# Fan-Luo/Legal-RAG

Measured on AMD Instinct MI355X. Metric: queries/sec + Recall@10 (hybrid top-10) on UCC-en, higher is better.
Workload: dtype f32 dense (long batches: fp16 first pass, candidates re-scored in f32) / f64 bm25+fusion; 1 GPU; UCC-en 591 chunks, dense(768-d FlatIP)+BM25 hybrid fusion top-10 (BASELINE configs[1]); unique_queries=1168, top_k=10, fusion=rrf_norm_blend w=0.6/0.4 alpha=0.5 rrf_k=60 min_final=0.2

## Files before the change

### legal-rag_amd/csrc/fuse.hip

```cpp
#include "fuse_core.hpp"

#include <cfloat>
#include <cmath>
#include <cstdlib>
#include <cstring>
#include <vector>

namespace amdr {

constexpr int kFuseMax = 3 * AMDR_MAX_K;

__global__ __launch_bounds__(64) void fuse_kernel(amdr_fuse_params_t P, ChanIn c0, ChanIn c1, ChanIn c2, int max_out,
                                                  long long* __restrict__ out_ids, double* __restrict__ out_vals,
                                                  int* __restrict__ out_mask, int* __restrict__ out_count) {
  extern __shared__ __attribute__((aligned(16))) unsigned char fsm[];
  long long* uid = reinterpret_cast<long long*>(fsm);
  double* sc = reinterpret_cast<double*>(uid + max_out);
  double* tot = sc + max_out;
  int* pos0 = reinterpret_cast<int*>(tot + max_out);
  int* pos[3] = {pos0, pos0 + max_out, pos0 + 2 * max_out};
  const int lane = threadIdx.x;
  const int qi = blockIdx.x;
  const ChanIn ch[3] = {c0, c1, c2};
  const double w[3] = {P.w_dense, P.w_bm25, P.w_colbert};

  int n[3];
  double lo[3], hi[3];
#pragma unroll
  for (int c = 0; c < 3; ++c) {
    int cnt = 0;
    double mn = INFINITY, mx = -INFINITY;
    for (int j = lane; j < ch[c].k; j += 64) {
      if (ch[c].ids[(size_t)qi * ch[c].k + j] >= 0) {
        cnt++;
        double s = chan_score(ch[c], qi, j);
        mn = fmin(mn, s);
        mx = fmax(mx, s);
      }
    }
    n[c] = wave_allsum_i32(cnt);
    lo[c] = wave_min(mn);
    hi[c] = wave_max(mx);
  }

  int U = 0;
#pragma unroll
  for (int c = 0; c < 3; ++c) {
    const int U0 = U;
    for (int base = 0; base < n[c]; base += 64) {
      const int j = base + lane;
      const bool v = j < n[c];
      long long my = v ? chan_uid(ch[c], qi, j) : -1;
      int f = -1;
      if (v)
        for (int u = 0; u < U0; ++u)
          if (uid[u] == my) {
            f = u;
            break;
          }
      const bool isnew = v && f < 0;
      const unsigned long long m = __ballot(isnew);
      const unsigned long long lt = (lane == 0) ? 0ull : (m & (~0ull >> (64 - lane)));
      const int idx = isnew ? U + __popcll(lt) : f;
      if (isnew) {
        uid[idx] = my;
        pos[0][idx] = -1;
        pos[1][idx] = -1;
        pos[2][idx] = -1;
      }
      lds_sync();
      if (v) pos[c][idx] = j;
      U += __popcll(m);
      lds_sync();
    }
  }

  const bool wrrf = (P.method == AMDR_FUSE_WRRF);
  double rmn = INFINITY, rmx = -INFINITY;
  for (int u = lane; u < U; u += 64) {
    double t = 0.0;
#pragma unroll
    for (int c = 0; c < 3; ++c) {
      int p = pos[c][u];
      if (p >= 0) {
        double wc = wrrf ? w[c] : 1.0;
        double v = wc * (1.0 / (double)(P.rrf_k + p + 1));
        t = t + v;
      }
    }
    tot[u] = t;
    rmn = fmin(rmn, t);
    rmx = fmax(rmx, t);
  }
  rmn = wave_min(rmn);
  rmx = wave_max(rmx);
  const bool rdeg = (rmx - rmn < 1e-12);

  FuseCtx X;
  X.rmn = rmn;
  X.rmx = rmx;
  X.rdeg = rdeg;
  X.wrrf = wrrf;
#pragma unroll
  for (int c = 0; c < 3; ++c) {
    X.w[c] = w[c];
    X.lo[c] = lo[c];
    X.hi[c] = hi[c];
  }
  auto eval = [&](int u, double (&val)[AMDR_FUSE_NVALS], int& mk) {
    const int pp[3] = {pos[0][u], pos[1][u], pos[2][u]};
    fuse_eval(P, X, tot[u], pp, [&](int c, int p) { return chan_score(ch[c], qi, p); }, val, mk);
  };

  int kept = 0;
  const size_t obase = (size_t)qi * max_out;
  if (U <= 64) {
    double val[AMDR_FUSE_NVALS];
    int mk = 0;
    const int u = lane;
    if (u < U) {
      eval(u, val, mk);
      sc[u] = val[AMDR_FV_SCORE];
    }
    lds_sync();
    if (u < U) {
      const double s = val[AMDR_FV_SCORE];
      int r = 0;
      for (int v2 = 0; v2 < U; ++v2) {
        const double o = sc[v2];
        r += (o > s) || (o == s && v2 < u);
      }
      if (s >= P.min_final_score) kept++;
      out_ids[obase + r] = uid[u];
      out_mask[obase + r] = mk;
#pragma unroll
      for (int x = 0; x < AMDR_FUSE_NVALS; ++x) out_vals[(obase + r) * AMDR_FUSE_NVALS + x] = val[x];
    }
  } else {
    for (int u = lane; u < U; u += 64) {
      double val[AMDR_FUSE_NVALS];
      int mk;
      eval(u, val, mk);
      sc[u] = val[AMDR_FV_SCORE];
    }
    lds_sync();
    for (int u = lane; u < U; u += 64) {
      double val[AMDR_FUSE_NVALS];
      int mk;
      eval(u, val, mk);
      const double s = val[AMDR_FV_SCORE];
      int r = 0;
      for (int v2 = 0; v2 < U; ++v2) {
        const double o = sc[v2];
        r += (o > s) || (o == s && v2 < u);
      }
      if (s >= P.min_final_score) kept++;
      out_ids[obase + r] = uid[u];
      out_mask[obase + r] = mk;
#pragma unroll
      for (int x = 0; x < AMDR_FUSE_NVALS; ++x) out_vals[(obase + r) * AMDR_FUSE_NVALS + x] = val[x];
    }
  }
  kept = wave_allsum_i32(kept);
  for (int r = U + lane; r < max_out; r += 64) {
    out_ids[obase + r] = -1;
    out_mask[obase + r] = 0;
    for (int x = 0; x < AMDR_FUSE_NVALS; ++x) out_vals[(obase + r) * AMDR_FUSE_NVALS + x] = 0.0;
  }
  if (lane == 0) out_count[qi] = kept;
}

template <int W>
__global__ __launch_bounds__(64) void fuse_packed_kernel(amdr_fuse_params_t P, ChanIn c0, ChanIn c1, ChanIn c2, int nq,
                                                         int max_out, long long* __restrict__ out_ids,
                                                         double* __restrict__ out_vals, int* __restrict__ out_mask,
                                                         int* __restrict__ out_count) {
  FusePre none;
  none.have[0] = none.have[1] = none.have[2] = false;
  fuse_packed_body<W, false>(P, c0, c1, c2, nq, max_out, out_ids, out_vals, out_mask, out_count, none, blockIdx.x * (64 / W));
}

static void launch_fuse(const amdr_fuse_params_t& P, const ChanIn& c0, const ChanIn& c1, const ChanIn& c2, int nq,
                        int max_out, long long* ids, double* vals, int* mask, int* count, hipStream_t st) {
  if (max_out <= 16)
    hipLaunchKernelGGL(fuse_packed_kernel<16>, dim3((nq + 3) / 4), dim3(64), 0, st, P, c0, c1, c2, nq, max_out, ids, vals,
                       mask, count);
  else if (max_out <= 32)
    hipLaunchKernelGGL(fuse_packed_kernel<32>, dim3((nq + 1) / 2), dim3(64), 0, st, P, c0, c1, c2, nq, max_out, ids, vals,
                       mask, count);
  else
    hipLaunchKernelGGL(fuse_kernel, dim3(nq), dim3(64), (size_t)max_out * 36, st, P, c0, c1, c2, max_out, ids, vals, mask,
                       count);
}

__global__ __launch_bounds__(64) void rerank_blend_kernel(int max_out, const int* __restrict__ count,
                                                          long long* __restrict__ ids, double* __restrict__ vals,
                                                          int* __restrict__ mask, const double* __restrict__ ce_raw,
                                                          int top_n, double beta, double* __restrict__ out_rerank) {
  extern __shared__ __attribute__((aligned(16))) unsigned char smem[];
  double* svals = reinterpret_cast<double*>(smem);
  double* snew = svals + (size_t)max_out * AMDR_FUSE_NVALS;
  double* snorm = snew + max_out;
  long long* sids = reinterpret_cast<long long*>(snorm + max_out);
  int* smask = reinterpret_cast<int*>(sids + max_out);
  int* spre = smask + max_out;
  const int lane = threadIdx.x, qi = blockIdx.x;
  const size_t base = (size_t)qi * max_out;
  const int cnt = count[qi];
  const int n = cnt < top_n ? cnt : top_n;
  const double nan = __longlong_as_double(0x7ff8000000000000ll);

  for (int r = lane; r < max_out; r += 64) {
    out_rerank[(base + r) * 2 + 0] = nan;
    out_rerank[(base + r) * 2 + 1] = nan;
  }
  if (n <= 0) return;

  double mn = INFINITY, mx = -INFINITY;
  for (int j = lane; j < n; j += 64) {
    double r = ce_raw[(size_t)qi * top_n + j];
    mn = fmin(mn, r);
    mx = fmax(mx, r);
  }
  mn = wave_min(mn);
  mx = wave_max(mx);
  const bool deg = (mx - mn < 1e-12);

  for (int j = lane; j < cnt; j += 64) {
    for (int x = 0; x < AMDR_FUSE_NVALS; ++x) svals[(size_t)j * AMDR_FUSE_NVALS + x] = vals[(base + j) * AMDR_FUSE_NVALS + x];
    sids[j] = ids[base + j];
    smask[j] = mask[base + j];
    double s = svals[(size_t)j * AMDR_FUSE_NVALS + AMDR_FV_SCORE];
    if (j < n) {
      double raw = ce_raw[(size_t)qi * top_n + j];
      double nm = deg ? 0.0 : (raw - mn) / (mx - mn);
      snorm[j] = nm;
      s = (1 - beta) * s + beta * nm;
    }
    snew[j] = s;
  }
  lds_sync();
  for (int j = lane; j < cnt; j += 64) {
    int p = j;
    if (j < n) {
      const double nm = snorm[j];
      p = 0;
      for (int i = 0; i < n; ++i) {
        const double o = snorm[i];
        p += (o > nm) || (o == nm && i < j);
      }
    }
    spre[j] = p;
  }
  lds_sync();
  for (int j = lane; j < cnt; j += 64) {
    const double s = snew[j];
    const int pj = spre[j];
    int r = 0;
    for (int i = 0; i < cnt; ++i) {
      const double o = snew[i];
      r += (o > s) || (o == s && spre[i] < pj);
    }
    ids[base + r] = sids[j];
    mask[base + r] = smask[j];
    for (int x = 0; x < AMDR_FUSE_NVALS; ++x) vals[(base + r) * AMDR_FUSE_NVALS + x] = svals[(size_t)j * AMDR_FUSE_NVALS + x];
    vals[(base + r) * AMDR_FUSE_NVALS + AMDR_FV_SCORE] = s;
    if (j < n) {
      out_rerank[(base + r) * 2 + 0] = ce_raw[(size_t)qi * top_n + j];
      out_rerank[(base + r) * 2 + 1] = snorm[j];
    }
  }
}

static size_t rerank_lds(int max_out) {
  return (size_t)max_out * (AMDR_FUSE_NVALS + 2) * sizeof(double) + (size_t)max_out * sizeof(long long) +
         (size_t)max_out * 2 * sizeof(int);
}

int dense_fuse_plain_launch(const FuseTail& t, int q0, int m, int kd, const float* dense_scores, const int64_t* dense_ids,
                            hipStream_t st) {
  const FuseTailArgs a = fuse_tail_args(t, q0, kd, dense_scores, dense_ids);
  launch_fuse(*t.p, a.c0, a.c1, ChanIn::none(), m, a.mo, a.ids, a.vals, a.mask, a.count, st);
  AMDR_HIP(hipGetLastError());
  return AMDR_OK;
}

}

using namespace amdr;

namespace {

int fuse_check(const amdr_fuse_params_t* p, int nq, int kd, int kb, int kc) {
  AMDR_REQUIRE(p != nullptr, "fuse: null params");
  AMDR_REQUIRE(p->method >= 0 && p->method <= 3, "fuse: unknown method %d", p->method);
  AMDR_REQUIRE(nq >= 0, "fuse: nq=%d", nq);
  AMDR_REQUIRE(kd >= 0 && kd <= AMDR_MAX_K && kb >= 0 && kb <= AMDR_MAX_K && kc >= 0 && kc <= AMDR_MAX_K,
               "fuse: channel depth outside [0,%d]", AMDR_MAX_K);
  AMDR_REQUIRE(kd + kb + kc >= 1, "fuse: all channels empty (max_out would be 0)");
  return AMDR_OK;
}

}

namespace {
struct Arena {
  char* base = nullptr;
  size_t cap = 0, used = 0;
  int device = -1;
  ~Arena() {
    if (base) (void)hipFree(base);
  }
  int begin(int dev, size_t total) {
    if (dev != device || total > cap) {
      if (base) (void)hipFree(base);
      base = nullptr;
      cap = 0;
      size_t want = total < (1u << 20) ? (1u << 20) : total;
      AMDR_HIP(hipMalloc((void**)&base, want));
      cap = want;
      device = dev;
    }
    used = 0;
    return AMDR_OK;
  }
  void* take(size_t bytes) {
    void* p = base + used;
    used += (bytes + 255) & ~(size_t)255;
    return p;
  }
};
inline size_t pad256(size_t b) { return (b + 255) & ~(size_t)255; }
Arena& arena() {
  static thread_local Arena a;
  return a;
}
}

namespace {
struct Pack {
  std::vector<char>& buf;
  size_t used = 0;
  explicit Pack(std::vector<char>& b) : buf(b) {}
  size_t add(const void* src, size_t bytes) {
    size_t off = used;
    used += pad256(bytes);
    if (buf.size() < used) buf.resize(used);
    if (src && bytes) memcpy(buf.data() + off, src, bytes);
    return off;
  }
};
std::vector<char>& host_block() {
  static thread_local std::vector<char> b;
  return b;
}
}

namespace amdr {
__global__ __launch_bounds__(256) void fuse_compact_kernel(const long long* __restrict__ ids, const double* __restrict__ vals,
                                                           const int* __restrict__ mask, const int* __restrict__ count,
                                                           int nq, int max_out, int w, long long* __restrict__ out_rows,
                                                           double* __restrict__ out_scores, int* __restrict__ out_mask,
                                                           int* __restrict__ out_count) {
  const long i = (long)blockIdx.x * 256 + threadIdx.x;
  if (i >= (long)nq * w) return;
  const int q = (int)(i / w), j = (int)(i - (long)q * w);
  const int c = count[q] < w ? count[q] : w;
  const bool keep = j < c;
  const size_t src = (size_t)q * max_out + j;
  out_rows[i] = keep ? ids[src] : -1ll;
  out_scores[i] = keep ? vals[src * AMDR_FUSE_NVALS + AMDR_FV_SCORE] : 0.0;
  out_mask[i] = keep ? mask[src] : 0;
  if (j == 0) out_count[q] = c;
}
}

extern "C" {

int amdr_fuse_device(const amdr_fuse_params_t* p, int32_t nq, const int64_t* dense_ids, const float* dense_scores,
                     int32_t kd, const int64_t* dense_row2uid, const int64_t* bm25_ids, const double* bm25_scores,
                     int32_t kb, const int64_t* bm25_row2uid, const int64_t* colbert_ids, const float* colbert_scores,
                     int32_t kc, const int64_t* colbert_row2uid, int64_t* out_ids, double* out_vals,
                     int32_t* out_mask, int32_t* out_count, int32_t device, void* stream) {
  int rc = fuse_check(p, nq, kd, kb, kc);
  if (rc) return rc;
  AMDR_REQUIRE((kd == 0 || (dense_ids && dense_scores)) && (kb == 0 || (bm25_ids && bm25_scores)) &&
                   (kc == 0 || (colbert_ids && colbert_scores)),
               "fuse: null channel buffer");
  AMDR_REQUIRE(nq == 0 || (out_ids && out_vals && out_mask && out_count), "fuse: null output");
  if (nq == 0) return AMDR_OK;
  AMDR_HIP(hipSetDevice(device));
  ChanIn c0{(const long long*)dense_ids, dense_scores, (const long long*)dense_row2uid, kd, 0};
  ChanIn c1{(const long long*)bm25_ids, bm25_scores, (const long long*)bm25_row2uid, kb, 1};
  ChanIn c2{(const long long*)colbert_ids, colbert_scores, (const long long*)colbert_row2uid, kc, 0};
  launch_fuse(*p, c0, c1, c2, nq, kd + kb + kc, (long long*)out_ids, out_vals, out_mask, out_count, (hipStream_t)stream);
  AMDR_HIP(hipGetLastError());
  return AMDR_OK;
}

int amdr_rerank_blend_device(int32_t nq, int32_t max_out, const int32_t* count, int64_t* ids, double* vals,
                             int32_t* mask, const double* ce_raw, int32_t top_n, double beta, double* out_rerank,
                             int32_t device, void* stream) {
  AMDR_REQUIRE(nq >= 0 && max_out >= 1 && max_out <= kFuseMax, "rerank_blend: bad sizes");
  AMDR_REQUIRE(top_n >= 1, "rerank_blend: top_n=%d", top_n);
  AMDR_REQUIRE(nq == 0 || (count && ids && vals && mask && ce_raw && out_rerank), "rerank_blend: null buffer");
  if (nq == 0) return AMDR_OK;
  AMDR_HIP(hipSetDevice(device));
  size_t lds = rerank_lds(max_out);
  if (lds > 48 * 1024)
    AMDR_HIP(hipFuncSetAttribute((const void*)rerank_blend_kernel, hipFuncAttributeMaxDynamicSharedMemorySize, (int)lds));
  hipLaunchKernelGGL(rerank_blend_kernel, dim3(nq), dim3(64), lds, (hipStream_t)stream, max_out, count,
                     (long long*)ids, vals, mask, ce_raw, top_n, beta, out_rerank);
  AMDR_HIP(hipGetLastError());
  return AMDR_OK;
}

int amdr_fuse_compact_device(int32_t nq, int32_t max_out, int32_t w, const int64_t* ids, const double* vals,
                             const int32_t* mask, const int32_t* count, int64_t* out_rows, double* out_scores,
                             int32_t* out_mask, int32_t* out_count, int32_t device, void* stream) {
  AMDR_REQUIRE(nq >= 0 && max_out >= 1 && w >= 1 && w <= max_out, "fuse_compact: bad sizes (max_out=%d w=%d)", max_out, w);
  if (nq == 0) return AMDR_OK;
  AMDR_REQUIRE(ids && vals && mask && count && out_rows && out_scores && out_mask && out_count, "fuse_compact: null buffer");
  AMDR_HIP(hipSetDevice(device));
  const long total = (long)nq * w;
  hipLaunchKernelGGL(amdr::fuse_compact_kernel, dim3((unsigned)((total + 255) / 256)), dim3(256), 0, (hipStream_t)stream,
                     (const long long*)ids, vals, mask, count, nq, max_out, w, (long long*)out_rows, out_scores, out_mask,
                     out_count);
  AMDR_HIP(hipGetLastError());
  return AMDR_OK;
}

int amdr_fuse(const amdr_fuse_params_t* p, int32_t nq, const int64_t* dense_ids, const double* dense_scores, int32_t kd,
              const int64_t* bm25_ids, const double* bm25_scores, int32_t kb, const int64_t* colbert_ids,
              const double* colbert_scores, int32_t kc, int64_t* out_ids, double* out_vals, int32_t* out_mask,
              int32_t* out_count) {
  int rc = fuse_check(p, nq, kd, kb, kc);
  if (rc) return rc;
  if (nq == 0) return AMDR_OK;
  AMDR_REQUIRE((kd == 0 || (dense_ids && dense_scores)) && (kb == 0 || (bm25_ids && bm25_scores)) &&
                   (kc == 0 || (colbert_ids && colbert_scores)) && out_ids && out_vals && out_mask && out_count,
               "fuse: null buffer");
  int dev = 0;
  AMDR_HIP(hipGetDevice(&dev));
  const size_t q = (size_t)nq, mo = (size_t)(kd + kb + kc);
  Pack in(host_block());
  const size_t o_di = in.add(dense_ids, q * kd * 8), o_ds = in.add(dense_scores, q * kd * 8);
  const size_t o_bi = in.add(bm25_ids, q * kb * 8), o_bs = in.add(bm25_scores, q * kb * 8);
  const size_t o_ci = in.add(colbert_ids, q * kc * 8), o_cs = in.add(colbert_scores, q * kc * 8);
  const size_t in_bytes = in.used;
  const size_t o_oi = in_bytes, o_ov = o_oi + pad256(q * mo * 8), o_om = o_ov + pad256(q * mo * AMDR_FUSE_NVALS * 8),
               o_oc = o_om + pad256(q * mo * 4), total = o_oc + pad256(q * 4);
  if ((rc = arena().begin(dev, total))) return rc;
  char* d = arena().base;
  hipStream_t st = nullptr;
  std::vector<char>& hb = host_block();
  if (hb.size() < total) hb.resize(total);
  AMDR_HIP(hipMemcpyAsync(d, hb.data(), in_bytes, hipMemcpyHostToDevice, st));
  ChanIn c0{(const long long*)(d + o_di), d + o_ds, nullptr, kd, 1};
  ChanIn c1{(const long long*)(d + o_bi), d + o_bs, nullptr, kb, 1};
  ChanIn c2{(const long long*)(d + o_ci), d + o_cs, nullptr, kc, 1};
  launch_fuse(*p, c0, c1, c2, nq, (int)mo, (long long*)(d + o_oi), (double*)(d + o_ov), (int*)(d + o_om),
              (int*)(d + o_oc), st);
  AMDR_HIP(hipGetLastError());
  AMDR_HIP(hipMemcpyAsync(hb.data() + o_oi, d + o_oi, total - o_oi, hipMemcpyDeviceToHost, st));
  AMDR_HIP(hipStreamSynchronize(st));
  memcpy(out_ids, hb.data() + o_oi, q * mo * 8);
  memcpy(out_vals, hb.data() + o_ov, q * mo * AMDR_FUSE_NVALS * 8);
  memcpy(out_mask, hb.data() + o_om, q * mo * 4);
  memcpy(out_count, hb.data() + o_oc, q * 4);
  return AMDR_OK;
}

int amdr_rerank_blend(int32_t nq, int32_t max_out, const int32_t* count, int64_t* ids, double* vals, int32_t* mask,
                      const double* ce_raw, int32_t top_n, double beta, double* out_rerank) {
  AMDR_REQUIRE(nq >= 0 && max_out >= 1 && max_out <= kFuseMax && top_n >= 1, "rerank_blend: bad sizes");
  if (nq == 0) return AMDR_OK;
  AMDR_REQUIRE(count && ids && vals && mask && ce_raw && out_rerank, "rerank_blend: null buffer");
  int dev = 0, rc;
  AMDR_HIP(hipGetDevice(&dev));
  const size_t q = (size_t)nq, mo = (size_t)max_out;
  Pack in(host_block());
  const size_t o_c = in.add(count, q * 4), o_r = in.add(ce_raw, q * top_n * 8);
  const size_t o_i = in.add(ids, q * mo * 8), o_v = in.add(vals, q * mo * AMDR_FUSE_NVALS * 8),
               o_m = in.add(mask, q * mo * 4);
  const size_t in_bytes = in.used;
  const size_t o_o = in_bytes, total = o_o + pad256(q * mo * 16);
  if ((rc = arena().begin(dev, total))) return rc;
  char* d = arena().base;
  hipStream_t st = nullptr;
  std::vector<char>& hb = host_block();
  if (hb.size() < total) hb.resize(total);
  AMDR_HIP(hipMemcpyAsync(d, hb.data(), in_bytes, hipMemcpyHostToDevice, st));
  rc = amdr_rerank_blend_device(nq, max_out, (const int32_t*)(d + o_c), (int64_t*)(d + o_i), (double*)(d + o_v),
                                (int32_t*)(d + o_m), (const double*)(d + o_r), top_n, beta, (double*)(d + o_o), dev, st);
  if (rc) return rc;
  AMDR_HIP(hipMemcpyAsync(hb.data() + o_i, d + o_i, total - o_i, hipMemcpyDeviceToHost, st));
  AMDR_HIP(hipStreamSynchronize(st));
  memcpy(ids, hb.data() + o_i, q * mo * 8);
  memcpy(vals, hb.data() + o_v, q * mo * AMDR_FUSE_NVALS * 8);
  memcpy(mask, hb.data() + o_m, q * mo * 4);
  memcpy(out_rerank, hb.data() + o_o, q * mo * 16);
  return AMDR_OK;
}


}
```

### legal-rag_amd/csrc/fuse_core.hpp

```cpp
#pragma once
#include "common.hpp"
#include "topk.hpp"

#include <cmath>

namespace amdr {

__device__ __forceinline__ double wave_min(double v) { return wave_allmin_f64(v); }
__device__ __forceinline__ double wave_max(double v) { return wave_allmax_f64(v); }
__device__ __forceinline__ void lds_sync() {
  __builtin_amdgcn_fence(__ATOMIC_ACQ_REL, "wavefront");
  __builtin_amdgcn_wave_barrier();
}

struct ChanIn {
  const long long* ids;
  const void* scores;
  const long long* row2uid;
  int k;
  int is_f64;
  __host__ __device__ static ChanIn none() { return ChanIn{nullptr, nullptr, nullptr, 0, 0}; }
};

__device__ __forceinline__ double chan_score(const ChanIn& c, int qi, int j) {
  size_t off = (size_t)qi * c.k + j;
  return c.is_f64 ? ((const double*)c.scores)[off] : (double)((const float*)c.scores)[off];
}
__device__ __forceinline__ long long chan_uid(const ChanIn& c, int qi, int j) {
  long long id = c.ids[(size_t)qi * c.k + j];
  if (id >= 0 && c.row2uid) id = c.row2uid[id];
  return id;
}

struct FuseCtx {
  double rmn, rmx;
  bool rdeg, wrrf;
  double w[3], lo[3], hi[3];
};
template <class ScoreAt>
__device__ __forceinline__ void fuse_eval(const amdr_fuse_params_t& P, const FuseCtx& X, double t, const int (&pos)[3],
                                          ScoreAt&& score_at, double (&val)[AMDR_FUSE_NVALS], int& mk) {
  const double rrf_norm = X.rdeg ? 0.0 : (t - X.rmn) / (X.rmx - X.rmn);
  double nrm[3], raw[3], wt[3];
  mk = 0;
#pragma unroll
  for (int c = 0; c < 3; ++c) {
    const int p = pos[c];
    nrm[c] = 0.0;
    raw[c] = 0.0;
    if (p >= 0) {
      mk |= (1 << c);
      const double s = score_at(c, p);
      nrm[c] = (X.hi[c] - X.lo[c] < 1e-12) ? 0.0 : (s - X.lo[c]) / (X.hi[c] - X.lo[c]);
      const double wc = X.wrrf ? X.w[c] : 1.0;
      raw[c] = wc * (1.0 / (double)(P.rrf_k + p + 1));
    }
    wt[c] = X.w[c] * nrm[c];
  }
  const double wsum = (wt[0] + wt[1]) + wt[2];
  double score, con[3] = {0.0, 0.0, 0.0};
  if (P.method == AMDR_FUSE_WEIGHTED_SUM) {
    score = wsum;
#pragma unroll
    for (int c = 0; c < 3; ++c) con[c] = wt[c];
  } else if (P.method == AMDR_FUSE_RRF || P.method == AMDR_FUSE_WRRF) {
    score = rrf_norm;
    const double mass = score;
    if (!(mass <= 0.0 || t <= 1e-18)) {
#pragma unroll
      for (int c = 0; c < 3; ++c)
        if (pos[c] >= 0) con[c] = mass * raw[c] / t;
    }
  } else {
    score = P.alpha * rrf_norm + (1.0 - P.alpha) * wsum;
#pragma unroll
    for (int c = 0; c < 3; ++c) con[c] = 0.0 + (1.0 - P.alpha) * wt[c];
    const double mass = P.alpha * rrf_norm;
    if (!(mass <= 0.0 || t <= 1e-18)) {
#pragma unroll
      for (int c = 0; c < 3; ++c)
        if (pos[c] >= 0) con[c] = con[c] + mass * raw[c] / t;
    }
  }
  val[AMDR_FV_SCORE] = score;
  val[AMDR_FV_RRF_NORM] = rrf_norm;
  val[AMDR_FV_WSUM] = wsum;
  val[AMDR_FV_NORM_DENSE] = nrm[0];
  val[AMDR_FV_NORM_BM25] = nrm[1];
  val[AMDR_FV_NORM_COLBERT] = nrm[2];
  val[AMDR_FV_CONTRIB_DENSE] = con[0];
  val[AMDR_FV_CONTRIB_BM25] = con[1];
  val[AMDR_FV_CONTRIB_COLBERT] = con[2];
}

struct FusePre {
  bool have[3];
  long long id[3];
  double s[3];
  __device__ __forceinline__ void dense_bm25(const ChanIn& c1, int q, int sl, bool live) {
    have[0] = have[1] = true;
    have[2] = false;
    id[1] = -1;
    s[1] = 0.0;
    if (live && sl < c1.k) {
      id[1] = c1.ids[(size_t)q * c1.k + sl];
      s[1] = chan_score(c1, q, sl);
    }
  }
  __device__ __forceinline__ void dense(const C32& c, bool valid) {
    id[0] = valid ? c.id() : -1ll;
    s[0] = valid ? (double)c.score() : 0.0;
  }
  __device__ __forceinline__ void bm25(const C64& c, bool valid) {
    id[1] = valid ? c.idv : -1ll;
    s[1] = valid ? unord64(c.key) : 0.0;
  }
};
template <int W, bool PRE>
__device__ __forceinline__ void fuse_packed_body(const amdr_fuse_params_t& P, const ChanIn& c0, const ChanIn& c1,
                                                 const ChanIn& c2, int nq, int max_out, long long* __restrict__ out_ids,
                                                 double* __restrict__ out_vals, int* __restrict__ out_mask,
                                                 int* __restrict__ out_count, const FusePre& pre, int qbase) {
  constexpr int G = 64 / W;
  __shared__ long long s_uid[G][W];
  __shared__ double s_sc[G][W];
  __shared__ double s_chs[G][3][W];
  __shared__ int s_pos[G][3][W];
  const int lane = threadIdx.x, seg = lane / W, sl = lane % W;
  const int qi = qbase + seg;
  const bool live = qi < nq;
  const ChanIn ch[3] = {c0, c1, c2};
  const double w[3] = {P.w_dense, P.w_bm25, P.w_colbert};
  const unsigned long long seg_bits = (W == 64) ? ~0ull : (((1ull << (W & 63)) - 1ull) << (seg * W));
  long long* uid = s_uid[seg];
  double* sc = s_sc[seg];

  int n[3] = {0, 0, 0};
  double lo[3] = {INFINITY, INFINITY, INFINITY}, hi[3] = {-INFINITY, -INFINITY, -INFINITY};
  long long my_uid[3] = {-1, -1, -1};
#pragma unroll
  for (int c = 0; c < 3; ++c) {
    if (ch[c].k == 0) continue;
    const int j = sl;
    const bool inr = live && j < ch[c].k;
    long long id = -1;
    double s = 0.0;
    if (PRE && pre.have[c]) {
      if (inr) {
        id = pre.id[c];
        s = pre.s[c];
      }
    } else if (inr) {
      id = ch[c].ids[(size_t)qi * ch[c].k + j];
      s = chan_score(ch[c], qi, j);
    }
    const bool has = inr && id >= 0;
    if (!has) s = 0.0;
    if (has && ch[c].row2uid) id = ch[c].row2uid[id];
    my_uid[c] = has ? id : -1;
    s_chs[seg][c][sl] = s;
    const unsigned long long hm = __ballot(has) & seg_bits;
    n[c] = __popcll(hm);
    const double nxt = __shfl_down(s, 1);
    const bool in_order = !(has && sl + 1 < n[c]) || s >= nxt;
    const bool prefix = hm == (seg_bits & ((n[c] >= 64 ? ~0ull : ((1ull << n[c]) - 1ull)) << (seg * W)));
    if (__ballot(!in_order || !prefix) == 0ull) {
      const int first = seg * W, last = seg * W + (n[c] > 0 ? n[c] - 1 : 0);
      const double top = __shfl(s, first), bot = __shfl(s, last);
      hi[c] = n[c] > 0 ? top : -(double)INFINITY;
      lo[c] = n[c] > 0 ? bot : (double)INFINITY;
    } else {
      lo[c] = seg_allmin_f64<W>(has ? s : (double)INFINITY);
      hi[c] = seg_allmax_f64<W>(has ? s : -(double)INFINITY);
    }
  }

  int U = 0;
#pragma unroll
  for (int c = 0; c < 3; ++c) {
    if (ch[c].k == 0) continue;
    const int U0 = U;
    const bool v = sl < n[c];
    const long long my = my_uid[c];
    int f = -1;
    int u_end = 0;
#pragma unroll
    for (int g = 0; g < G; ++g) {
      const int ug = __builtin_amdgcn_readlane(U0, g * W);
      u_end = ug > u_end ? ug : u_end;
    }
    for (int u0 = 0; u0 < u_end; u0 += 4) {
      long long e[4];
#pragma unroll
      for (int i = 0; i < 4; ++i) e[i] = uid[(u0 + i) & (W - 1)];
#pragma unroll
      for (int i = 0; i < 4; ++i) f = (u0 + i < U0 && e[i] == my) ? u0 + i : f;
    }
    f = v ? f : -1;
    const bool isnew = v && f < 0;
    const unsigned long long m = __ballot(isnew) & seg_bits;
    const unsigned long long lt = m & ((1ull << lane) - 1ull);
    const int idx = isnew ? U + __popcll(lt) : f;
    if (isnew) {
      uid[idx] = my;
      s_pos[seg][0][idx] = -1;
      s_pos[seg][1][idx] = -1;
      s_pos[seg][2][idx] = -1;
    }
    lds_sync();
    if (v) s_pos[seg][c][idx] = sl;
    U += __popcll(m);
    lds_sync();
  }

  const bool wrrf = (P.method == AMDR_FUSE_WRRF);
  const int u = sl;
  const bool act = u < U;
  int pp[3] = {-1, -1, -1};
  double t = 0.0;
  if (act) {
#pragma unroll
    for (int c = 0; c < 3; ++c) {
      pp[c] = s_pos[seg][c][u];
      if (pp[c] >= 0) {
        const double wc = wrrf ? w[c] : 1.0;
        const double v = wc * (1.0 / (double)(P.rrf_k + pp[c] + 1));
        t = t + v;
      }
    }
  }
  FuseCtx X;
  X.rmn = seg_allmin_f64<W>(act ? t : (double)INFINITY);
  X.rmx = seg_allmax_f64<W>(act ? t : -(double)INFINITY);
  X.rdeg = (X.rmx - X.rmn < 1e-12);
  X.wrrf = wrrf;
#pragma unroll
  for (int c = 0; c < 3; ++c) {
    X.w[c] = w[c];
    X.lo[c] = lo[c];
    X.hi[c] = hi[c];
  }

  double val[AMDR_FUSE_NVALS];
  int mk = 0;
  if (act) {
    fuse_eval(P, X, t, pp, [&](int c, int p) { return s_chs[seg][c][p]; }, val, mk);
    sc[u] = val[AMDR_FV_SCORE];
  }
  lds_sync();
  int kept = 0;
  const size_t obase = (size_t)qi * max_out;
  if (act) {
    const double s = val[AMDR_FV_SCORE];
    int r = 0;
    for (int v2 = 0; v2 < U; ++v2) {
      const double o = sc[v2];
      r += (o > s) || (o == s && v2 < u);
    }
    if (s >= P.min_final_score) kept = 1;
    out_ids[obase + r] = uid[u];
    out_mask[obase + r] = mk;
#pragma unroll
    for (int x = 0; x < AMDR_FUSE_NVALS; ++x) out_vals[(obase + r) * AMDR_FUSE_NVALS + x] = val[x];
  } else if (live && u < max_out) {
    out_ids[obase + u] = -1;
    out_mask[obase + u] = 0;
#pragma unroll
    for (int x = 0; x < AMDR_FUSE_NVALS; ++x) out_vals[(obase + u) * AMDR_FUSE_NVALS + x] = 0.0;
  }
  kept = __popcll(__ballot(kept != 0) & seg_bits);
  if (live && sl == 0) out_count[qi] = kept;
}

struct FuseTailArgs {
  ChanIn c0, c1;
  int mo;
  long long* ids;
  double* vals;
  int* mask;
  int* count;
};
inline FuseTailArgs fuse_tail_args(const FuseTail& t, int q0, int kd, const float* dense_scores, const int64_t* dense_ids) {
  const int mo = kd + t.kb;
  return FuseTailArgs{ChanIn{(const long long*)dense_ids, dense_scores, (const long long*)t.dense_row2uid, kd, 0},
                      ChanIn{(const long long*)(t.kb ? t.bm25_ids + (size_t)q0 * t.kb : nullptr),
                             t.kb ? (const void*)(t.bm25_scores + (size_t)q0 * t.kb) : nullptr,
                             (const long long*)t.bm25_row2uid, t.kb, 1},
                      mo, (long long*)(t.out_ids + (size_t)q0 * mo), t.out_vals + (size_t)q0 * mo * AMDR_FUSE_NVALS,
                      t.out_mask + (size_t)q0 * mo, t.out_count + q0};
}

}
```

Before: 151.9 million queries/s.

## Stage fused output records in LDS and write them with coalesced vector stores

The fuse and rerank-blend kernels used to scatter each output record (ids, mask, vals) straight to global memory at its rank position, one strided write per thread. Records are now placed in an LDS staging buffer at their rank slot and copied to global memory as contiguous 16-byte vector stores in chunks of 32 rows. The packed kernel reuses its dead shared arrays for the stage. The cost is extra LDS traffic and wave barriers per chunk, plus a NaN-fill path that keeps unranked slots defined.

```diff
diff --git a/legal-rag_amd/csrc/fuse.hip b/legal-rag_amd/csrc/fuse.hip
--- a/legal-rag_amd/csrc/fuse.hip
+++ b/legal-rag_amd/csrc/fuse.hip
@@ -1,5 +1,6 @@
 #include "fuse_core.hpp"
 
+#include <algorithm>
 #include <cfloat>
 #include <cmath>
 #include <cstdlib>
@@ -123,19 +124,23 @@
       sc[u] = val[AMDR_FV_SCORE];
     }
     lds_sync();
+    int r = -1;
+    long long rec_uid = -1;
     if (u < U) {
       const double s = val[AMDR_FV_SCORE];
-      int r = 0;
+      r = 0;
       for (int v2 = 0; v2 < U; ++v2) {
         const double o = sc[v2];
         r += (o > s) || (o == s && v2 < u);
       }
       if (s >= P.min_final_score) kept++;
-      out_ids[obase + r] = uid[u];
-      out_mask[obase + r] = mk;
-#pragma unroll
-      for (int x = 0; x < AMDR_FUSE_NVALS; ++x) out_vals[(obase + r) * AMDR_FUSE_NVALS + x] = val[x];
-    }
+      rec_uid = uid[u];
+    }
+    lds_sync();
+    const bool nan_rank = __ballot(u < U && val[AMDR_FV_SCORE] != val[AMDR_FV_SCORE]) != 0ull;
+    for (int c0 = 0; c0 < U; c0 += kRecChunk)
+      store_record_chunk(fsm, lane, r >= c0 ? r - c0 : -1, U - c0 < kRecChunk ? U - c0 : kRecChunk, nan_rank, rec_uid, mk, val,
+                         out_ids, out_vals, out_mask, obase + c0);
   } else {
     for (int u = lane; u < U; u += 64) {
       double val[AMDR_FUSE_NVALS];
@@ -189,8 +194,8 @@
     hipLaunchKernelGGL(fuse_packed_kernel<32>, dim3((nq + 1) / 2), dim3(64), 0, st, P, c0, c1, c2, nq, max_out, ids, vals,
                        mask, count);
   else
-    hipLaunchKernelGGL(fuse_kernel, dim3(nq), dim3(64), (size_t)max_out * 36, st, P, c0, c1, c2, max_out, ids, vals, mask,
-                       count);
+    hipLaunchKernelGGL(fuse_kernel, dim3(nq), dim3(64), std::max((size_t)max_out * 36, (size_t)kRecStageBytes), st, P, c0, c1,
+                       c2, max_out, ids, vals, mask, count);
 }
 
 __global__ __launch_bounds__(64) void rerank_blend_kernel(int max_out, const int* __restrict__ count,
@@ -204,6 +209,8 @@
   long long* sids = reinterpret_cast<long long*>(snorm + max_out);
   int* smask = reinterpret_cast<int*>(sids + max_out);
   int* spre = smask + max_out;
+  int* sinv = spre + max_out;
+  unsigned char* stage = smem + ((size_t)max_out * 108 + 15) / 16 * 16;
   const int lane = threadIdx.x, qi = blockIdx.x;
   const size_t base = (size_t)qi * max_out;
   const int cnt = count[qi];
@@ -251,6 +258,7 @@
       }
     }
     spre[j] = p;
+    sinv[j] = -1;
   }
   lds_sync();
   for (int j = lane; j < cnt; j += 64) {
@@ -261,20 +269,35 @@
       const double o = snew[i];
       r += (o > s) || (o == s && spre[i] < pj);
     }
-    ids[base + r] = sids[j];
-    mask[base + r] = smask[j];
-    for (int x = 0; x < AMDR_FUSE_NVALS; ++x) vals[(base + r) * AMDR_FUSE_NVALS + x] = svals[(size_t)j * AMDR_FUSE_NVALS + x];
-    vals[(base + r) * AMDR_FUSE_NVALS + AMDR_FV_SCORE] = s;
+    sinv[r] = j;
     if (j < n) {
       out_rerank[(base + r) * 2 + 0] = ce_raw[(size_t)qi * top_n + j];
       out_rerank[(base + r) * 2 + 1] = snorm[j];
     }
   }
+  lds_sync();
+  for (int c0 = 0; c0 < cnt; c0 += kRecChunk) {
+    const int rows = cnt - c0 < kRecChunk ? cnt - c0 : kRecChunk;
+    double val[AMDR_FUSE_NVALS];
+    long long id = -1;
+    int mk = 0;
+    if (lane < rows) {
+      const int ji = sinv[c0 + lane];
+      const int j = ji >= 0 ? ji : c0 + lane;
+#pragma unroll
+      for (int x = 0; x < AMDR_FUSE_NVALS; ++x) val[x] = svals[(size_t)j * AMDR_FUSE_NVALS + x];
+      if (ji >= 0) val[AMDR_FV_SCORE] = snew[j];
+      id = sids[j];
+      mk = smask[j];
+    }
+    store_record_chunk(stage, lane, lane < rows ? lane : -1, rows, false, id, mk, val, ids, vals, mask, base + c0);
+  }
 }
 
 static size_t rerank_lds(int max_out) {
-  return (size_t)max_out * (AMDR_FUSE_NVALS + 2) * sizeof(double) + (size_t)max_out * sizeof(long long) +
-         (size_t)max_out * 2 * sizeof(int);
+  const size_t lists = (size_t)max_out * (AMDR_FUSE_NVALS + 2) * sizeof(double) + (size_t)max_out * sizeof(long long) +
+                       (size_t)max_out * 3 * sizeof(int);
+  return (lists + 15) / 16 * 16 + kRecStageBytes;
 }
 
 int dense_fuse_plain_launch(const FuseTail& t, int q0, int m, int kd, const float* dense_scores, const int64_t* dense_ids,
diff --git a/legal-rag_amd/csrc/fuse_core.hpp b/legal-rag_amd/csrc/fuse_core.hpp
--- a/legal-rag_amd/csrc/fuse_core.hpp
+++ b/legal-rag_amd/csrc/fuse_core.hpp
@@ -11,6 +11,61 @@
 __device__ __forceinline__ void lds_sync() {
   __builtin_amdgcn_fence(__ATOMIC_ACQ_REL, "wavefront");
   __builtin_amdgcn_wave_barrier();
+}
+
+constexpr int kRecChunk = 32;
+constexpr int kRecValBytes = kRecChunk * AMDR_FUSE_NVALS * 8;
+constexpr int kRecStageBytes = kRecValBytes + kRecChunk * 8 + kRecChunk * 4;
+typedef unsigned rec_u4 __attribute__((ext_vector_type(4)));
+typedef unsigned rec_u2 __attribute__((ext_vector_type(2)));
+__device__ __forceinline__ void wave_store_run(void* dst, const unsigned char* src, int bytes, int lane) {
+  unsigned char* d = static_cast<unsigned char*>(dst);
+  const unsigned mis = __builtin_amdgcn_readfirstlane((unsigned)(reinterpret_cast<uintptr_t>(d) & 15u));
+  int done;
+  if (mis == 0) {
+    const int n = bytes >> 4;
+#pragma clang loop unroll(disable)
+    for (int i = lane; i < n; i += 64) reinterpret_cast<rec_u4*>(d)[i] = reinterpret_cast<const rec_u4*>(src)[i];
+    done = n << 4;
+  } else if ((mis & 7u) == 0) {
+    const int n = bytes >> 3;
+#pragma clang loop unroll(disable)
+    for (int i = lane; i < n; i += 64) reinterpret_cast<rec_u2*>(d)[i] = reinterpret_cast<const rec_u2*>(src)[i];
+    done = n << 3;
+  } else {
+    done = 0;
+  }
+#pragma clang loop unroll(disable)
+  for (int i = (done >> 2) + lane; i < (bytes >> 2); i += 64)
+    reinterpret_cast<unsigned*>(d)[i] = reinterpret_cast<const unsigned*>(src)[i];
+}
+__device__ __forceinline__ void store_record_chunk(unsigned char* stage, int lane, int slot, int rows, bool fill, long long uid,
+                                                   int mk, const double (&val)[AMDR_FUSE_NVALS],
+                                                   long long* __restrict__ out_ids, double* __restrict__ out_vals,
+                                                   int* __restrict__ out_mask, size_t row0) {
+  double* sv = reinterpret_cast<double*>(stage);
+  long long* si = reinterpret_cast<long long*>(stage + kRecValBytes);
+  int* sm = reinterpret_cast<int*>(stage + kRecValBytes + kRecChunk * 8);
+  if (fill) {
+    if (lane < rows) {
+      si[lane] = -1;
+      sm[lane] = 0;
+#pragma unroll
+      for (int x = 0; x < AMDR_FUSE_NVALS; ++x) sv[lane * AMDR_FUSE_NVALS + x] = 0.0;
+    }
+    lds_sync();
+  }
+  if (slot >= 0 && slot < rows) {
+    si[slot] = uid;
+    sm[slot] = mk;
+#pragma unroll
+    for (int x = 0; x < AMDR_FUSE_NVALS; ++x) sv[slot * AMDR_FUSE_NVALS + x] = val[x];
+  }
+  lds_sync();
+  wave_store_run(out_vals + row0 * AMDR_FUSE_NVALS, stage, rows * AMDR_FUSE_NVALS * 8, lane);
+  wave_store_run(out_ids + row0, stage + kRecValBytes, rows * 8, lane);
+  wave_store_run(out_mask + row0, stage + kRecValBytes + kRecChunk * 8, rows * 4, lane);
+  lds_sync();
 }
 
 struct ChanIn {
@@ -122,10 +177,12 @@
                                                  double* __restrict__ out_vals, int* __restrict__ out_mask,
                                                  int* __restrict__ out_count, const FusePre& pre, int qbase) {
   constexpr int G = 64 / W;
-  __shared__ long long s_uid[G][W];
-  __shared__ double s_sc[G][W];
-  __shared__ double s_chs[G][3][W];
-  __shared__ int s_pos[G][3][W];
+  __shared__ __attribute__((aligned(16))) unsigned char s_raw[64 * (3 * 8 + 3 * 4 + 8 + 8)];
+  static_assert(sizeof(s_raw) >= (size_t)kRecStageBytes, "the record stage must fit in the dead arrays");
+  double (*s_chs)[3][W] = reinterpret_cast<double (*)[3][W]>(s_raw);
+  int (*s_pos)[3][W] = reinterpret_cast<int (*)[3][W]>(s_raw + 64 * 3 * 8);
+  long long (*s_uid)[W] = reinterpret_cast<long long (*)[W]>(s_raw + 64 * (3 * 8 + 3 * 4));
+  double (*s_sc)[W] = reinterpret_cast<double (*)[W]>(s_raw + 64 * (3 * 8 + 3 * 4 + 8));
   const int lane = threadIdx.x, seg = lane / W, sl = lane % W;
   const int qi = qbase + seg;
   const bool live = qi < nq;
@@ -242,6 +299,8 @@
   }
 
   double val[AMDR_FUSE_NVALS];
+#pragma unroll
+  for (int x = 0; x < AMDR_FUSE_NVALS; ++x) val[x] = 0.0;
   int mk = 0;
   if (act) {
     fuse_eval(P, X, t, pp, [&](int c, int p) { return s_chs[seg][c][p]; }, val, mk);
@@ -249,25 +308,26 @@
   }
   lds_sync();
   int kept = 0;
-  const size_t obase = (size_t)qi * max_out;
+  int r = u;
+  long long rec_uid = -1;
   if (act) {
     const double s = val[AMDR_FV_SCORE];
-    int r = 0;
+    r = 0;
     for (int v2 = 0; v2 < U; ++v2) {
       const double o = sc[v2];
       r += (o > s) || (o == s && v2 < u);
     }
     if (s >= P.min_final_score) kept = 1;
-    out_ids[obase + r] = uid[u];
-    out_mask[obase + r] = mk;
-#pragma unroll
-    for (int x = 0; x < AMDR_FUSE_NVALS; ++x) out_vals[(obase + r) * AMDR_FUSE_NVALS + x] = val[x];
-  } else if (live && u < max_out) {
-    out_ids[obase + u] = -1;
-    out_mask[obase + u] = 0;
-#pragma unroll
-    for (int x = 0; x < AMDR_FUSE_NVALS; ++x) out_vals[(obase + u) * AMDR_FUSE_NVALS + x] = 0.0;
-  }
+    rec_uid = uid[u];
+  }
+  lds_sync();
+  const int n_live = nq - qbase < G ? nq - qbase : G;
+  const int rows_all = __builtin_amdgcn_readfirstlane(n_live > 0 ? n_live * max_out : 0);
+  const int my_row = (live && r < max_out) ? seg * max_out + r : -1;
+  const bool nan_rank = __ballot(act && val[AMDR_FV_SCORE] != val[AMDR_FV_SCORE]) != 0ull;
+  for (int c0 = 0; c0 < rows_all; c0 += kRecChunk)
+    store_record_chunk(s_raw, lane, my_row >= c0 ? my_row - c0 : -1, rows_all - c0 < kRecChunk ? rows_all - c0 : kRecChunk,
+                       nan_rank, rec_uid, mk, val, out_ids, out_vals, out_mask, (size_t)qbase * max_out + c0);
   kept = __popcll(__ballot(kept != 0) & seg_bits);
   if (live && sl == 0) out_count[qi] = kept;
 }
```

New measurement: 153.4 million queries/s, median of 6. Within noise of the previous version (+1.0%).
